# UCSC-nanopore-cgl/margin

Measured on AMD Instinct MI355X. Metric: het-sites x reads phased/sec (30x ONT synthetic chunks, end to end: every merge level + final sweep), higher is better.
Workload: dtype int32

## Files before the change

### include/margin_rphmm.h

```cpp
#ifndef MARGIN_RPHMM_H_
#define MARGIN_RPHMM_H_

#include <stddef.h>
#include <stdint.h>

#ifdef __cplusplus
extern "C" {
#endif

#define MRP_OK 0
#define MRP_ERR_ARG 1
#define MRP_ERR_NO_DEVICE 2
#define MRP_ERR_HIP 3
#define MRP_ERR_NOMEM 4
#define MRP_ERR_UNSUPPORTED 5
#define MRP_ERR_LOOKUP 6

#define MRP_ALLELE_LOG_PROB_BITS 8
#define MRP_MAX_READ_PARTITIONING_DEPTH 64
#define MRP_MAX_ALLELES 16

#define MRP_FLAG_MAX_NOT_SUM 1u
#define MRP_FLAG_INCLUDE_ANCESTOR_SUB_PROB 2u

// ... 1 lines not shown
typedef struct mrp_chunk mrp_chunk;
typedef struct mrp_batch mrp_batch;

const char *mrp_last_error(void);
const char *mrp_version(void);
#define MRP_ABI_VERSION 6
int mrp_abi_version(void);
int mrp_device_count(void);

int mrp_context_create(int device, mrp_context **out);
void mrp_context_destroy(mrp_context *ctx);
int mrp_context_synchronize(mrp_context *ctx);
int mrp_context_trim(mrp_context *ctx);
int mrp_runtime_init(void);
int mrp_context_set_phase_groups(mrp_context *ctx, int groups);
int mrp_context_set_test_hooks(mrp_context *ctx, int hooks);
int mrp_set_host_threads(int n);

int mrp_chunk_create(mrp_context *ctx, int64_t n_sites, const uint32_t *allele_number,
                     const uint16_t *substitution_log_probs, const uint16_t *allele_prior_log_probs,
                     const uint8_t *profile_pool, int64_t pool_bytes, mrp_chunk **out);
void mrp_chunk_destroy(mrp_chunk *chunk);

typedef struct mrp_hmm_job {
    const mrp_chunk *chunk;
    int32_t n_columns;
    uint32_t flags;
    const int32_t *col_ref_start;
    const int32_t *col_length;
    const int32_t *col_depth;
// ... 552 lines not shown
```

### margin_amd/capi.py

```python
from __future__ import annotations

import ctypes as C
import os
import time
from typing import Dict, List, Optional, Sequence

import numpy as np

_HERE = os.path.dirname(os.path.abspath(__file__))
LIB_PATH = os.environ.get("MRP_LIB_OVERRIDE") or os.path.join(_HERE, "lib", "libmargin_rphmm.so")

MRP_OK = 0
MRP_ERR_ARG, MRP_ERR_NO_DEVICE, MRP_ERR_HIP, MRP_ERR_NOMEM, MRP_ERR_UNSUPPORTED, MRP_ERR_LOOKUP = 1, 2, 3, 4, 5, 6
WIDE_MAX_WIDTH, WIDE_MAX_CELLS = 32768, 1 << 31
FLAG_MAX_NOT_SUM = 1
FLAG_INCLUDE_ANCESTOR_SUB_PROB = 2

ABI_VERSION = 6

EXPORTED_SYMBOLS = [
    "mrp_last_error", "mrp_version", "mrp_abi_version", "mrp_runtime_init", "mrp_device_count", "mrp_context_create", "mrp_context_destroy",
    "mrp_context_synchronize", "mrp_context_trim", "mrp_hmm_split", "mrp_hmm_split_where_phasing_is_uncertain", "mrp_context_set_phase_groups", "mrp_context_set_test_hooks", "mrp_set_host_threads", "mrp_chunk_create", "mrp_chunk_destroy", "mrp_fb_run", "mrp_batch_create",
    "mrp_batch_add", "mrp_batch_upload", "mrp_batch_launch", "mrp_batch_download", "mrp_batch_destroy",
    "mrp_batch_stats", "mrp_count_bit_vectors", "mrp_emissions", "mrp_get_rp_hmms", "mrp_hmm_destroy", "mrp_free",
    "mrp_hmm_view", "mrp_hmm_forward_backward", "mrp_hmm_prune", "mrp_hmm_forward_trace_back", "mrp_phase_reads",
    "mrp_phase_result_destroy", "mrp_get_rp_hmms_resident", "mrp_phase_reads_many", "mrp_reference_from_bubbles",
    "mrp_profile_seqs_from_bubbles", "mrp_assign_reads_to_haplotypes", "mrp_stitch_create", "mrp_stitch_destroy",
    "mrp_stitch_chunk", "mrp_stitch_size", "mrp_stitch_lookup", "mrp_phase_sets", "mrp_binomial_p_value", "mrp_binomial_coefficient",
    "mrp_symbols_from_chars", "mrp_pair_hmm_reverse_complement", "mrp_band_diagonals", "mrp_forward_probabilities",
    "mrp_allele_read_supports", "mrp_kmer_alignment_anchors", "mrp_phase_chunks_on_devices", "mrp_queue_plan", "mrp_queue_dry_run", "mrp_queue_create", "mrp_queue_destroy",
    "mrp_queue_phase_chunks", "mrp_partition_reads_by_haplotype", "mrp_phase_variants_from_tagged_reads", "mrp_phase_string_chunks",
    "mrp_extract_read_substrings", "mrp_string_chunk_from_extracted", "mrp_string_chunk_units", "mrp_queue_phase_string_chunks",
    "mrp_phase_string_chunks_on_devices", "mrp_phase_string_chunks_with_filtered", "mrp_queue_phase_string_chunks_with_filtered",
    "mrp_phase_string_chunks_with_filtered_on_devices", "mrp_haptag_sites_from_extracted", "mrp_haplotag_aligned_chunks",
    "mrp_kmer_alignment_anchors_many", "mrp_phase_aligned_chunks", "mrp_string_chunk_rest_from_extracted", "mrp_equal_substring_classes",
    "mrp_phase_aligned_chunks_with_filtered", "mrp_aligned_chunk_units", "mrp_queue_phase_aligned_chunks",
    "mrp_queue_phase_aligned_chunks_with_filtered", "mrp_phase_aligned_chunks_on_devices", "mrp_phase_aligned_chunks_with_filtered_on_devices",
# ... 269 lines not shown
    vp, i64, i32, u32 = C.c_void_p, C.c_int64, C.c_int32, C.c_uint32
    P = C.POINTER
    L.mrp_last_error.restype = C.c_char_p
    L.mrp_version.restype = C.c_char_p
    L.mrp_abi_version.restype = C.c_int
    if L.mrp_abi_version() != ABI_VERSION:
        raise MrpError(f"libmargin_rphmm.so speaks ABI {L.mrp_abi_version()}, this binding was transcribed from ABI {ABI_VERSION} of include/margin_rphmm.h")
    L.mrp_device_count.restype = C.c_int
    L.mrp_context_create.argtypes = [C.c_int, P(vp)]
    L.mrp_context_destroy.argtypes = [vp]
    L.mrp_context_destroy.restype = None
    L.mrp_context_synchronize.argtypes = [vp]
    L.mrp_context_trim.argtypes = [vp]
    L.mrp_context_set_phase_groups.argtypes = [vp, C.c_int]
    L.mrp_context_set_test_hooks.argtypes = [vp, C.c_int]
    L.mrp_set_host_threads.argtypes = [C.c_int]
    L.mrp_chunk_create.argtypes = [vp, i64, vp, vp, vp, vp, i64, P(vp)]
    L.mrp_chunk_destroy.argtypes = [vp]
    L.mrp_chunk_destroy.restype = None
    L.mrp_fb_run.argtypes = [vp, i64, P(HmmJob)]
    L.mrp_batch_create.argtypes = [vp, P(vp)]
    L.mrp_batch_add.argtypes = [vp, P(HmmJob)]
    L.mrp_batch_upload.argtypes = [vp]
    L.mrp_batch_launch.argtypes = [vp]
    L.mrp_batch_download.argtypes = [vp]
    L.mrp_batch_destroy.argtypes = [vp]
    L.mrp_batch_destroy.restype = None
    L.mrp_batch_stats.argtypes = [vp, P(LaunchStats)]
    L.mrp_count_bit_vectors.argtypes = [vp, vp, i32, i32, i32, vp, vp]
    L.mrp_emissions.argtypes = [vp, vp, i32, i32, i32, vp, u32, i64, vp, vp]
# ... 99 lines not shown
    def __init__(self, device: int = 0):
        L = load()
        h = C.c_void_p()
        _check(L.mrp_context_create(device, C.byref(h)))
        self.h = h

    def synchronize(self):
        _check(load().mrp_context_synchronize(self.h))

    def trim(self):
        _check(load().mrp_context_trim(self.h))

    def set_phase_groups(self, groups: int):
        _check(load().mrp_context_set_phase_groups(self.h, groups))

    def set_test_hooks(self, hooks: int):
        _check(load().mrp_context_set_test_hooks(self.h, hooks))

    def set_wide_pairs(self, on):
        _check(load().mrp_context_set_wide_pairs(self.h, int(bool(on))))

    def wide_pair_count(self):
        pairs, cells = C.c_int64(), C.c_int64()
        _check(load().mrp_context_wide_pair_count(self.h, C.byref(pairs), C.byref(cells)))
        return pairs.value, cells.value

    def close(self):
        if self.h:
            load().mrp_context_destroy(self.h)
            self.h = None
# ... 1400 lines not shown
```

### margin_amd/csrc/mrp_batch.cpp

```cpp
#include <hip/hip_runtime.h>

#include <algorithm>
#include <array>
#include <cstdio>
#include <cstdlib>
#include <cstring>
#include <ctime>
#include <mutex>
#include <new>
#include <vector>

#include "mrp_internal.h"
#include "mrp_level_order.h"

extern "C" {

int mrp_batch_create(mrp_context *ctx, mrp_batch **out) {
    if (!ctx || !out) return mrp_set_error(MRP_ERR_ARG, "mrp_batch_create: bad arguments");
    mrp_batch *b = new (std::nothrow) mrp_batch();
    if (!b) return mrp_set_error(MRP_ERR_NOMEM, "out of host memory");
    b->ctx = ctx;
    b->bind_pool(&ctx->pool);
    *out = b;
    return MRP_OK;
// ... 361 lines not shown
    HostVec<uint32_t>().swap(b->cell_next);
    HostVec<uint32_t>().swap(b->cell_prev);
    HostVec<uint32_t>().swap(b->cell_np);
    b->uploaded = true;
    return MRP_OK;
}

int mrp_batch_launch(mrp_batch *b) {
    if (!b) return mrp_set_error(MRP_ERR_ARG, "batch is NULL");
    if (!b->uploaded) {
        int rc = mrp_batch_upload(b);
        if (rc != MRP_OK) return rc;
    }
    mrp_context *ctx = b->ctx;
    HIP_TRY(hipSetDevice(ctx->device));
    hipStream_t s = ctx->stream;
    const MrpBatchDev &d = b->dev;
    hipStream_t ps = s;
    const size_t slot = (size_t) (b->n_launches % mrp_batch::EV_RING);
    if (slot >= b->ev_ring.size()) {
        std::array<hipEvent_t, 5> fresh{};
        for (auto &ev : fresh) HIP_TRY(hipEventCreate(&ev));
        b->ev_ring.push_back(fresh);
    }
    const std::array<hipEvent_t, 5> &ev = b->ev_ring[slot];
    if (b->n_launches >= mrp_batch::EV_RING) HIP_TRY(hipEventSynchronize(ev[2]));
    if (ps != s && ctx->last_emission) HIP_TRY(hipStreamWaitEvent(ps, ctx->last_emission, 0));
    HIP_TRY(hipEventRecord(ev[0], ps));
    HIP_TRY(mrp_launch_planes(d, ps));
    if (b->resident && mrp_dup('p')) HIP_TRY(mrp_launch_planes(d, ps));
    HIP_TRY(hipEventRecord(ev[1], ps));
// ... 266 lines not shown
```

### margin_amd/csrc/mrp_context.cpp

```cpp
#include <hip/hip_runtime.h>

#include <atomic>
#include <cstdarg>
#include <cstdio>
#include <cstdlib>
#include <mutex>
#include <new>

#include "mrp_internal.h"

static thread_local char g_err[512] = "";

extern "C" {

int mrp_set_error(int code, const char *fmt, ...) {
    va_list ap;
    va_start(ap, fmt);
    vsnprintf(g_err, sizeof(g_err), fmt, ap);
    va_end(ap);
    return code;
}

const char *mrp_last_error(void) { return g_err; }
const char *mrp_version(void) { return "margin_rphmm 0.5.0 gfx950"; }
int mrp_abi_version(void) { return MRP_ABI_VERSION; }

int mrp_runtime_init(void) {
    return MRP_OK;
}

int mrp_device_count(void) {
    int n = 0;
    if (hipGetDeviceCount(&n) != hipSuccess) return 0;
    return n;
}

int mrp_context_device(const mrp_context *ctx) { return ctx->device; }
void mrp_warn_hw_queues_once(int concurrent_batches) {
    static std::atomic<int> said{0};
    if (concurrent_batches <= 2 || getenv("MRP_QUIET")) return;
    const char *q = getenv("GPU_MAX_HW_QUEUES");
    const int have = q ? atoi(q) : 4;
    if (have >= 2 * concurrent_batches || have >= 16) return;
    if (said.exchange(1)) return;
    fprintf(stderr, "margin_rphmm: %d concurrent batches (two streams each) on %d hardware queues (GPU_MAX_HW_QUEUES%s): their kernels share "
                    "queues and serialize (MRP_QUIET silences this line)\n",
            concurrent_batches, have, q ? "" : " unset, the runtime's default");
}

int mrp_context_set_grouped(mrp_context *ctx, int grouped) { const int was = ctx->grouped ? 1 : 0; ctx->grouped = grouped != 0; return was; }
void mrp_context_set_concurrent_batches(mrp_context *ctx, int n) { ctx->concurrent_batches = n < 1 ? 1 : n; }
int mrp_context_calls_sharing_device(const mrp_context *ctx) { return ctx->calls_sharing_device; }
int64_t mrp_context_device_budget(mrp_context *ctx) {
    if (ctx->pool.device < 0 || hipSetDevice(ctx->device) != hipSuccess) return 0;
    const size_t b = DevPoolRegistry::get().budget_of(ctx->pool.device);
    return b > (size_t) 1 << 62 ? 0 : (int64_t) b;
}
// ... 3 lines not shown
    for (mrp_context *s_ : ctx->siblings) n += s_->pool.oom_local.load();
    return n;
}
void mrp_context_pool_bytes(mrp_context *ctx, int64_t *cached, int64_t *device_held) {
    { std::lock_guard<std::mutex> lock(ctx->pool.mu); *cached = (int64_t) ctx->pool.cached_bytes; }
    *device_held = ctx->pool.device >= 0 ? (int64_t) DevPoolRegistry::get().held[ctx->pool.device].load() : 0;
}
mrp_context *mrp_context_sibling(mrp_context *ctx, int i) {
    std::lock_guard<std::mutex> lock(ctx->sibling_mu);
    while ((int) ctx->siblings.size() <= i) {
        mrp_context *s = nullptr;
        if (mrp_context_create(ctx->device, &s) != MRP_OK) return nullptr;
        s->phase_groups = 1;
        s->grouped = true;
        s->test_hooks = ctx->test_hooks;
        ctx->siblings.push_back(s);
    }
    return ctx->siblings[(size_t) i];
}
int mrp_context_create(int device, mrp_context **out) {
    if (!out) return mrp_set_error(MRP_ERR_ARG, "mrp_context_create: out is NULL");
    *out = nullptr;
    int n = mrp_device_count();
    if (n <= 0) return mrp_set_error(MRP_ERR_NO_DEVICE, "no HIP device visible: the stRPHmm sweep has no CPU fallback");
    if (device < 0 || device >= n) return mrp_set_error(MRP_ERR_ARG, "device %d out of range (0..%d)", device, n - 1);
    HIP_TRY(hipSetDevice(device));
    mrp_context *ctx = new (std::nothrow) mrp_context();
    if (!ctx) return mrp_set_error(MRP_ERR_NOMEM, "out of host memory");
    ctx->device = device;
    ctx->pool.attach(device);
// ... 51 lines not shown
int mrp_context_set_phase_groups(mrp_context *ctx, int groups) {
    if (!ctx || groups < 0 || groups > 16) return mrp_set_error(MRP_ERR_ARG, "mrp_context_set_phase_groups: bad arguments");
    ctx->phase_groups = groups;
    return MRP_OK;
}
int mrp_context_phase_groups(const mrp_context *ctx) { return ctx->phase_groups; }
int mrp_context_set_test_hooks(mrp_context *ctx, int hooks) {
    if (!ctx || hooks < 0 || hooks > 127) return mrp_set_error(MRP_ERR_ARG, "mrp_context_set_test_hooks: bad arguments");
    if ((hooks & 4) && ctx->pool.device >= 0) DevPoolRegistry::get().inject_oom[ctx->pool.device].store(1);
    hooks &= ~4;
    ctx->test_hooks = hooks;
    for (mrp_context *s_ : ctx->siblings) s_->test_hooks = hooks;
    return MRP_OK;
}
int mrp_context_test_hooks(const mrp_context *ctx) { return ctx->test_hooks; }
int mrp_context_set_wide_pairs(mrp_context *ctx, int on) {
    if (!ctx) return mrp_set_error(MRP_ERR_ARG, "mrp_context_set_wide_pairs: context is NULL");
    ctx->wide_pairs = on != 0;
    return MRP_OK;
}
int mrp_context_wide_pair_count(mrp_context *ctx, int64_t *pairs_out, int64_t *cells_out) {
    if (!ctx) return mrp_set_error(MRP_ERR_ARG, "mrp_context_wide_pair_count: context is NULL");
    if (pairs_out) *pairs_out = ctx->wide_pair_count;
    if (cells_out) *cells_out = ctx->wide_cell_count;
    return MRP_OK;
}

}
```

### margin_amd/csrc/mrp_engine.cpp

```cpp
#include <hip/hip_runtime.h>

#include <cmath>
#include <cstdio>
#include <cstdlib>
#include <cstring>
#include <ctime>
#include <memory>
#include <new>
#include <vector>

#include "mrp_engine.h"
extern "C" void mrp_pool_set_tag(int t);
extern "C" void mrp_pool_set_weight(int ns_per_index);
#include "mrp_internal.h"
#include "mrp_level_order.h"

#define ENG_TRY(expr)                                                                                          \
    do {                                                                                                       \
        hipError_t e_ = (expr);                                                                                \
        if (e_ != hipSuccess) return mrp_set_error(MRP_ERR_HIP, "%s failed: %s", #expr, hipGetErrorString(e_)); \
    } while (0)

namespace {
struct Segment {
// ... 68 lines not shown
    void reset() { arrays.release(); on = false; }
};
}

struct mrp_engine_level_state {
    mrp_batch *b = nullptr;
    std::unique_ptr<Segment> seg;
    int seg_id = -1;
    mrp_xhmm *x = nullptr;
    int64_t n = 0;
    bool final_level = false;
    bool fused = false;
    bool units = false;
    bool any_pack = true, any_planes = true;
    bool deferred = false;
    HmmIndex ix;
    LevelOrder order;
    PruneParams pp{};
    DevBufGroup arrays;
    DevBuf<PlanCol> d_plan{arrays};
    DevBuf<XDesc> d_xd{arrays};
    DevBuf<mrp_xpar> d_par{arrays};
    DevBuf<int32_t> d_cstart{arrays}, d_croff{arrays};
    DevBuf<PlanHmm> d_phmm{arrays};
    DevBuf<uint16_t> d_dims{arrays};
    DevBuf<LayoutTot> d_tot{arrays};
    DevBuf<LayoutBase> d_base{arrays};
    DevBuf<int64_t> d_totals{arrays}, d_tile_sums{arrays};
    DevBuf<CrossCol> d_cc{arrays};
    DevBuf<PruneHmm> d_ph{arrays};
// ... 13 lines not shown
    hipError_t create_events() {
        hipError_t he = hipEventCreateWithFlags(&done, hipEventDisableTiming);
        if (he == hipSuccess) he = hipEventCreate(&lay0);
        if (he == hipSuccess) he = hipEventCreateWithFlags(&uploaded, hipEventDisableTiming);
        for (auto &e_ : ev)
            if (he == hipSuccess) he = hipEventCreate(&e_);
        return he;
    }
    void reset() {
        seg.reset();
        arrays.release();
        frag.reset();
        order.perm.clear();
        x = nullptr; n = 0;
        deferred = false;
        t = Timing{};
    }
    ~mrp_engine_level_state() {
        for (hipEvent_t e_ : {uploaded, done, lay0, ev[0], ev[1], ev[2], ev[3], ev[4]})
            if (e_) (void) hipEventDestroy(e_);
        if (b) mrp_batch_destroy(b);
    }
};

struct mrp_engine {
    mrp_context *ctx = nullptr;
    mrp_params params{};
    PruneParams pp{};
    DevBufGroup arrays;
    DevBuf<uint64_t> leaf_part{arrays};
// ... 17 lines not shown
};

static double eng_now() {
    timespec ts;
    clock_gettime(CLOCK_MONOTONIC, &ts);
    return 1e3 * ts.tv_sec + 1e-6 * ts.tv_nsec;
}

static int64_t level_bound_bytes(const mrp_engine_level_state *L) { return 16 * L->order.bound_cells + 8 * L->order.bound_merge; }

static void level_retire(mrp_engine *e, mrp_engine_level_state *L, bool complete = false) {
    if (!L) return;
    mrp_context *ctx = e->ctx;
    (void) hipSetDevice(ctx->device);
    if (!complete) {
        (void) ctx->wait_stream(ctx->stream);
        if (ctx->pre) (void) ctx->wait_stream(ctx->pre);
    }
    if (L->b) {
        L->b->recycle();
        e->spare.push_back(L->b);
        L->b = nullptr;
    }
    if (L->deferred) e->inflight_bytes -= level_bound_bytes(L);
    L->reset();
    e->spare_levels.push_back(L);
    ctx->pool.reclaim();
}

extern "C" {

int mrp_engine_create(mrp_context *ctx, const mrp_params *params, mrp_engine **out) {
    if (!ctx || !params || !out) return mrp_set_error(MRP_ERR_ARG, "mrp_engine_create: NULL argument");
    *out = nullptr;
    if (params->reserved != 0) return mrp_set_error(MRP_ERR_ARG, "mrp_params.reserved must be 0");
    if (!params->max_not_sum_transitions)
        return mrp_set_error(MRP_ERR_UNSUPPORTED, "the device-resident merge needs maxNotSumTransitions (integer posteriors)");
    const int64_t lim = std::max<int64_t>(params->min_partitions_in_a_column, params->max_partitions_in_a_column);
    if (lim < 1 || lim > MRP_PRUNE_MAX_S || params->min_partitions_in_a_column < 0)
        return mrp_set_error(MRP_ERR_UNSUPPORTED, "the device-resident merge keeps at most %d partitions per column", MRP_PRUNE_MAX_S);
    ENG_TRY(hipSetDevice(ctx->device));
    mrp_engine *e = new (std::nothrow) mrp_engine();
// ... 403 lines not shown
        if (n1 < 0 || n2 < 0 || n1 > cap || n2 > cap) return;
        memcpy(h.frag_sites, h_sites + f.site0, sizeof(FragSite) * (size_t) f.length);
        memcpy(h.frag_reads1, h_lists + 2 * f.list0, 4 * (size_t) n1);
        memcpy(h.frag_reads2, h_lists + 2 * f.list0 + cap, 4 * (size_t) n2);
        h.frag_n1 = n1; h.frag_n2 = n2; h.frag_done = 1;
    });
}

static int level_stage(mrp_engine *e, int64_t n, mrp_xhmm *x, bool final_level) {
    if (!e || n < 0 || (n > 0 && !x)) return mrp_set_error(MRP_ERR_ARG, "mrp_engine_level: bad arguments");
    if (e->staged) return mrp_set_error(MRP_ERR_ARG, "mrp_engine_level_stage: a staged level was not launched");
    if (n == 0) return MRP_OK;
    mrp_context *ctx = e->ctx;
    ENG_TRY(hipSetDevice(ctx->device));
    hipStream_t cs = nullptr;
    ENG_TRY(ctx->copy_stream(&cs));
    if (e->n_segs >= mrp_engine::MAX_SEGS) return mrp_set_error(MRP_ERR_UNSUPPORTED, "more than %d levels", mrp_engine::MAX_SEGS);
    std::unique_ptr<mrp_engine_level_state> L;
    int rc = level_take(e, n, x, final_level, L);
    if (rc != MRP_OK) return rc;
    L->t.begin = eng_now();
    L->x = x;
    L->n = n;
    L->final_level = final_level;
    L->fused = !final_level && !(ctx->test_hooks & 2);
    for (int64_t i = 0; i < n && L->fused; i++)
        if (x[i].flags & MRP_FLAG_INCLUDE_ANCESTOR_SUB_PROB) L->fused = false;
    L->units = L->fused && e->pp.pairs != 0 && !(ctx->test_hooks & (8 | 16));

    double tm[5];
    bool all_planes = true;
    tm[0] = eng_now();
    if ((rc = level_index(e, L.get(), cs, &all_planes)) != MRP_OK) return rc;
    tm[1] = eng_now();
    if ((rc = level_segment(e, L.get())) != MRP_OK) return rc;
    tm[2] = eng_now();
// ... 98 lines not shown
    if (rc == MRP_OK) {
        if (Lp->final_level) level_scatter_final(Lp);
        level_book_stats(e, Lp);
        e->segments.push_back(std::move(Lp->seg));
    }
    e->n_ended++;
    level_retire(e, Lp, complete);
    return rc;
}

static int level_finish(mrp_engine *e) {
    if (e->inflight.empty()) return MRP_OK;
    mrp_context *ctx = e->ctx;
    int rc = MRP_OK;
    hipError_t se = hipSetDevice(ctx->device);
    if (se == hipSuccess) se = ctx->wait_stream(ctx->stream);
    if (se != hipSuccess) rc = mrp_set_error(MRP_ERR_HIP, "hipStreamSynchronize failed: %s", hipGetErrorString(se));
    std::vector<mrp_engine_level_state *> all;
    all.swap(e->inflight);
    for (auto *Lp : all) {
        if (rc == MRP_OK) rc = level_finish_one(e, Lp, false);
        else { e->n_ended++; level_retire(e, Lp); }
    }
    return rc;
}

static int level_finish_ready(mrp_engine *e) {
    int rc = MRP_OK;
    while (rc == MRP_OK && !e->inflight.empty()) {
        mrp_engine_level_state *Lp = e->inflight.front();
        if (!Lp->done || hipEventQuery(Lp->done) != hipSuccess) { (void) hipGetLastError(); break; }
        e->inflight.erase(e->inflight.begin());
        rc = level_finish_one(e, Lp, true);
    }
    return rc;
}

static int launch_layout(mrp_engine *e, mrp_engine_level_state *L, hipStream_t s) {
    mrp_batch *b = L->b;
    LayoutOut lo{};
    lo.dims = L->d_dims.p; lo.tot = L->d_tot.p; lo.base = L->d_base.p; lo.totals = L->d_totals.p; lo.tile_sums = L->d_tile_sums.p;
    lo.hmms = b->d_hmms.p; lo.cols = b->d_cols.p; lo.scols = b->d_scols.p; lo.pcols = b->d_pcols.p; lo.tilecols = b->d_tilecols.p;
    lo.ccols = L->d_cc.p;
    ENG_TRY(hipStreamWaitEvent(s, L->uploaded, 0));
    ENG_TRY(hipEventRecord(L->lay0, s));
    ENG_TRY_DUP('l', mrp_launch_layout(L->d_plan.p, L->d_phmm.p, L->n, L->ix.total_cols, b->d_chunks.p, e->pp.S,
                                       (e->params.include_inverted_partitions ? MRP_XF_INVERTED : 0u) | (L->units ? MRP_XF_UNITS : 0u), lo, s));
    ENG_TRY(hipMemcpyAsync(L->res.totals, L->d_totals.p, 48, hipMemcpyDeviceToHost, s));
    return MRP_OK;
}

static constexpr int64_t DEFER_BYTES = (int64_t) 1024 << 20;
static constexpr size_t DEFER_LEVELS = 12;
static bool level_defers(const mrp_engine *e, const mrp_engine_level_state *L) {
    const int64_t bound_bytes = level_bound_bytes(L);
    return !(e->ctx->test_hooks & 32) && L->fused && !L->final_level && bound_bytes <= DEFER_BYTES &&
           e->inflight_bytes + bound_bytes <= 4 * DEFER_BYTES && e->inflight.size() < DEFER_LEVELS;
}

static int launch_size_batch(mrp_engine_level_state *L, int64_t cells, int64_t merge, int64_t tiles_fast, int64_t tiles) {
    mrp_batch *b = L->b;
    const int64_t n = L->n, total_cols = L->ix.total_cols, n_slots = L->ix.total_slots;
    b->n_cells_total = cells; b->n_merge = merge; b->n_slots = n_slots; b->n_tiles_dev = tiles; b->n_fast_tiles = tiles_fast;
    b->stats.n_cells = cells; b->stats.n_merge_cells = merge;
    b->stats.algorithmic_bytes = 24 * cells + 32 * merge + 8 * total_cols;
    const size_t nC = (size_t) cells;
    if (L->fused) { b->d_partition.release(); b->n_tiles_dev = 0; b->n_fast_tiles = 0; }
    else ENG_TRY(b->d_partition.alloc(nC));
    ENG_TRY(b->d_np.alloc(nC)); ENG_TRY(b->d_cost.alloc(nC));
    ENG_TRY(b->d_f32.alloc(nC)); ENG_TRY(b->d_b32.alloc(nC));
    ENG_TRY(b->d_mf32.alloc((size_t) merge)); ENG_TRY(b->d_mb32.alloc((size_t) merge));
    if (!L->fused) ENG_TRY(b->d_tiles.alloc((size_t) tiles));
// ... 63 lines not shown
        if (L->frag.on) { const int rc = L->frag.fetch(n, s); if (rc != MRP_OK) return rc; }
    }
    ENG_TRY(hipMemcpyAsync(L->res.err, L->d_err.p, 16, hipMemcpyDeviceToHost, s));
    ENG_TRY(hipMemcpyAsync(L->res.err_hmm, L->d_err_hmm.p, sizeof(int32_t) * (size_t) n, hipMemcpyDeviceToHost, s));
#if defined(PRUNE_EXP_CLOCK) || defined(PRUNE_EXP_CLOCK2) || defined(XE_CLOCK)
    ENG_TRY(hipMemcpyAsync(L->clk, L->d_err.p + 4, 96, hipMemcpyDeviceToHost, s));
#endif
    ENG_TRY(hipEventRecord(L->done, s));
    return MRP_OK;
}

static int level_launch_impl(mrp_engine *e, mrp_engine_level_state *L) {
    mrp_context *ctx = e->ctx;
    ENG_TRY(hipSetDevice(ctx->device));
    hipStream_t s = ctx->stream;
    const double t0 = eng_now();
    int rc = launch_layout(e, L, s);
    if (rc != MRP_OK) return rc;
    int64_t cells, merge, tiles_fast = 0, tiles = 0;
    if (level_defers(e, L)) {
        if ((rc = level_finish_ready(e)) != MRP_OK) return rc;
        cells = L->order.bound_cells; merge = L->order.bound_merge;
        L->deferred = true;
        e->inflight_bytes += level_bound_bytes(L);
    } else {
        if ((rc = level_finish(e)) != MRP_OK) return rc;
        ENG_TRY(ctx->wait_stream(s));
        L->t.react_ms = -eng_now();
        ctx->pool.reclaim();
        const int64_t *tot = L->res.totals;
// ... 35 lines not shown
```

### margin_amd/csrc/mrp_internal.h

```cpp
#ifndef MRP_INTERNAL_H_
#define MRP_INTERNAL_H_

#include <hip/hip_runtime.h>
#include <cstring>
#include <cstdlib>

#include <time.h>

#include <algorithm>
#include <array>
#include <atomic>
#include <functional>
#include <iterator>
#include <map>
#include <memory>
#include <new>
#include <type_traits>
#include <mutex>
#include <thread>
#include <utility>
#include <vector>

#include "../../include/margin_rphmm.h"
#include "mrp_device.h"
// ... 64 lines not shown
        }
        return b;
    }
    void forget_budget(int device) { if (device >= 0 && device < MAX_DEVICES) budget[device].store(0, std::memory_order_relaxed); }
    void shrink_budget(int device) {
        const size_t ours = held[device].load(std::memory_order_relaxed);
        size_t b = budget[device].load(std::memory_order_relaxed);
        if (ours > ((size_t) 1 << 30) && (b == 0 || ours < b)) budget[device].store(ours, std::memory_order_relaxed);
    }
    inline void trim_device(int device, DevPool *but);
};

struct DevPool {
    std::mutex mu;
    std::multimap<size_t, void *> free_blocks;
    std::vector<std::pair<size_t, void *>> pending;
    size_t cached_bytes = 0;
    size_t cache_limit = (size_t) 64 << 30;
    int device = -1;
    std::atomic<uint64_t> oom_local{0};
    void attach(int dev) {
        device = dev >= 0 && dev < DevPoolRegistry::MAX_DEVICES ? dev : -1;
        if (device < 0) return;
        DevPoolRegistry &r = DevPoolRegistry::get();
        std::lock_guard<std::mutex> lock(r.mu);
        r.pools.push_back(this);
    }
    void detach() {
        if (device < 0) return;
        DevPoolRegistry &r = DevPoolRegistry::get();
        std::lock_guard<std::mutex> lock(r.mu);
// ... 48 lines not shown
        if (e != hipSuccess && device >= 0) {
            (void) hipGetLastError();
            DevPoolRegistry::get().trim_device(device, this);
            e = hipMalloc(p, cls);
        }
        if (e == hipSuccess) held_add(cls);
        else if (e == hipErrorOutOfMemory && device >= 0) {
            DevPoolRegistry::get().oom_events[device].fetch_add(1, std::memory_order_relaxed);
            oom_local.fetch_add(1, std::memory_order_relaxed);
            DevPoolRegistry::get().shrink_budget(device);
        }
        return e;
    }
    void release(void *p, size_t cls) {
        std::lock_guard<std::mutex> lock(mu);
        pending.emplace_back(cls, p);
    }
    void reclaim() {
        std::lock_guard<std::mutex> lock(mu);
        for (auto &b : pending) {
            free_blocks.emplace(b.first, b.second);
            cached_bytes += b.first;
        }
        pending.clear();
        while ((cached_bytes > cache_limit || over_budget()) && !free_blocks.empty()) {
            auto it = std::prev(free_blocks.end());
            (void) hipFree(it->second);
            held_sub(it->first);
            cached_bytes -= it->first;
            free_blocks.erase(it);
        }
    }
    void trim() {
        std::lock_guard<std::mutex> lock(mu);
        for (auto &b : free_blocks) { (void) hipFree(b.second); held_sub(b.first); }
        free_blocks.clear();
        cached_bytes = 0;
    }
    void destroy() {
// ... 48 lines not shown
            (void) hipDeviceSynchronize();
            e = hipMemset(p, 0xA5, bytes);
            (void) hipDeviceSynchronize();
        }
#endif
        return e;
    }
    template <class A>
    hipError_t upload(const std::vector<T, A> &h, hipStream_t s) {
        hipError_t e = alloc(h.size());
        if (e != hipSuccess || h.empty()) return e;
        return hipMemcpyAsync(p, h.data(), h.size() * sizeof(T), hipMemcpyHostToDevice, s);
    }
};

struct mrp_context {
    int device = 0;
    hipStream_t stream = nullptr;
    hipStream_t aux[2] = {nullptr, nullptr};
    bool grouped = false;
    int concurrent_batches = 1;
    int calls_sharing_device = 1;
    hipError_t side_streams(hipStream_t *a0, hipStream_t *a1) {
        if (grouped) { *a0 = *a1 = stream; return hipSuccess; }
        for (int i = 0; i < 2; i++)
            if (!aux[i]) { const hipError_t e = hipStreamCreateWithFlags(&aux[i], hipStreamNonBlocking); if (e != hipSuccess) return e; }
        *a0 = aux[0]; *a1 = aux[1];
        return hipSuccess;
    }
    hipError_t copy_stream(hipStream_t *cs) {
        if (!pre) { const hipError_t e = hipStreamCreateWithFlags(&pre, hipStreamNonBlocking); if (e != hipSuccess) return e; }
        *cs = pre;
        return hipSuccess;
// ... 8 lines not shown
        timespec c0, c1, w0, w1;
        clock_gettime(CLOCK_THREAD_CPUTIME_ID, &c0); clock_gettime(CLOCK_MONOTONIC, &w0);
        const hipError_t e = wait_stream_impl(s);
        clock_gettime(CLOCK_THREAD_CPUTIME_ID, &c1); clock_gettime(CLOCK_MONOTONIC, &w1);
        wait_cpu_ms += 1e3 * (c1.tv_sec - c0.tv_sec) + 1e-6 * (c1.tv_nsec - c0.tv_nsec);
        wait_wall_ms += 1e3 * (w1.tv_sec - w0.tv_sec) + 1e-6 * (w1.tv_nsec - w0.tv_nsec);
        return e;
    }
    hipError_t wait_stream_impl(hipStream_t s) {
        if (!block_ev) {
            hipError_t e = hipEventCreateWithFlags(&block_ev, hipEventDisableTiming);
            if (e != hipSuccess) { block_ev = nullptr; return hipStreamSynchronize(s); }
        }
        hipError_t e = hipEventRecord(block_ev, s);
        if (e != hipSuccess) return e;
        for (;;) {
            e = hipEventQuery(block_ev);
            if (e != hipErrorNotReady) return e;
            timespec ts{0, 30000};
            nanosleep(&ts, nullptr);
        }
    }
    DevPool pool;
    int test_hooks = 0;
    int wide_pairs = 0;
    int64_t wide_pair_count = 0, wide_cell_count = 0;
    int phase_groups = 0;
    std::vector<mrp_context *> siblings;
    std::mutex sibling_mu;
    std::vector<struct mrp_engine_level_state *> spare_levels;
    std::vector<struct mrp_batch *> spare_batches;
};

struct mrp_chunk {
    mrp_context *ctx = nullptr;
    int64_t n_sites = 0, pool_bytes = 0;
// ... 60 lines not shown
struct mrp_batch {
    mrp_context *ctx = nullptr;
    std::mutex mu;
    std::vector<const mrp_chunk *> chunks;
    HostVec<DevHmm> hmms;
    HostVec<DevCol> cols;
    HostVec<int64_t> read_byte_off;
    HostVec<uint64_t> partition;
    HostVec<SweepCol> scols;
    HostVec<PlaneCol> pcols;
    HostVec<uint32_t> cell_next, cell_prev, cell_np;
    HostVec<EmitTile> tiles;
    int64_t n_fast_tiles = 0;
    int64_t n_tiles_dev = 0;
    std::function<hipError_t(hipStream_t)> pre_sweep;
    DevBufGroup arrays;
    DevBuf<TileCol> d_tilecols{arrays};
    bool need_wide = false;
    std::vector<JobOut> outs;
    int64_t n_merge = 0, n_slots = 0;
    int64_t n_cells_total = 0;
    bool resident = false;
    mrp_launch_stats stats{};
    std::vector<int32_t> order_wide, order_mid, order_narrow, order_f64, order_lse, order_lse_big, order_gen;
    int max_merge_wide = 1, max_merge_mid = 1, max_merge_narrow = 1, max_merge_lse = 1, max_merge_lse_big = 1;
    bool uploaded = false, launched = false;
    static constexpr int EV_RING = 32;
    std::vector<std::array<hipEvent_t, 5>> ev_ring;
    int64_t n_launches = 0, stats_mark = 0;
    DevBuf<DevHmm> d_hmms{arrays};
// ... 7 lines not shown
    DevBuf<double> d_f{arrays}, d_b{arrays}, d_mf{arrays}, d_mb{arrays}, d_total{arrays}, d_hmm_fb{arrays};
    DevBuf<int32_t> d_f32{arrays}, d_b32{arrays}, d_mf32{arrays}, d_mb32{arrays};
    DevBuf<int32_t> d_order_wide{arrays}, d_order_mid{arrays}, d_order_narrow{arrays}, d_order_f64{arrays}, d_order_lse{arrays}, d_order_lse_big{arrays},
        d_pack_list{arrays}, d_plane_list{arrays};
    DevBuf<EmitTile> d_tiles{arrays};
    MrpBatchDev dev{};
    void recycle() {
        arrays.release();
        chunks.clear(); hmms.clear(); cols.clear(); read_byte_off.clear(); partition.clear(); scols.clear(); pcols.clear();
        cell_next.clear(); cell_prev.clear(); cell_np.clear(); tiles.clear(); outs.clear();
        order_wide.clear(); order_mid.clear(); order_narrow.clear(); order_f64.clear(); order_lse.clear(); order_lse_big.clear(); order_gen.clear();
        n_fast_tiles = 0; n_tiles_dev = 0; need_wide = false; n_merge = 0; n_slots = 0; n_cells_total = 0; resident = false;
        stats = mrp_launch_stats{};
        max_merge_wide = max_merge_mid = max_merge_narrow = max_merge_lse = max_merge_lse_big = 1;
        uploaded = launched = false;
        n_launches = 0; stats_mark = 0;
        dev = MrpBatchDev{};
    }
    void bind_pool(DevPool *pl) { arrays.bind(pl); }
    MrpBatchDev view() const {
        MrpBatchDev d{};
        d.hmms = d_hmms.p; d.cols = d_cols.p; d.scols = d_scols.p; d.pcols = d_pcols.p; d.chunks = d_chunks.p; d.read_byte_off = d_read_byte_off.p;
        d.pack_list = d_pack_list.p; d.plane_list = d_plane_list.p; d.n_pack_list = (int64_t) d_pack_list.n; d.n_plane_list = (int64_t) d_plane_list.n;
        d.partition = d_partition.p; d.cell_np = d_np.p; d.cell_next = d_next.p; d.cell_prev = d_prev.p;
        d.planes = d_planes.p; d.slot_total = d_slot_total.p; d.slot_bytes = d_slot_bytes.p; d.cell_cost = d_cost.p;
        d.cell_f32 = d_f32.p; d.cell_b32 = d_b32.p; d.merge_f32 = d_mf32.p; d.merge_b32 = d_mb32.p;
        d.cell_f = d_f.p; d.cell_b = d_b.p; d.merge_f = d_mf.p; d.merge_b = d_mb.p; d.col_total = d_total.p; d.hmm_fb = d_hmm_fb.p;
        d.n_hmms = (int64_t) hmms.size(); d.n_cols = (int64_t) cols.size(); d.n_cells = n_cells_total; d.n_merge = n_merge; d.n_slots = n_slots;
        return d;
    }
// ... 105 lines not shown
```

### margin_amd/csrc/rphmm_host.h

```cpp
#ifndef RPHMM_HOST_H_
#define RPHMM_HOST_H_

#include <stdint.h>

#include "../../include/margin_rphmm.h"

#ifdef __cplusplus
extern "C" {
#endif

typedef struct mrp_chunk_host {
    int64_t n_sites;
    const uint32_t *allele_number;
    const uint32_t *allele_offset;
    const uint32_t *sub_offset;
    const uint16_t *sub;
    const uint16_t *prior;
    const uint8_t *pool;
    int64_t pool_bytes;
} mrp_chunk_host;

void mrp_chunk_host_view(const mrp_chunk *chunk, mrp_chunk_host *out);
mrp_context *mrp_chunk_context(const mrp_chunk *chunk);
void mrp_phase_group_assign(int64_t n_chunks, int G, int64_t total_sites, uint8_t *group_of);
int mrp_context_device(const mrp_context *ctx);
int mrp_context_set_grouped(mrp_context *ctx, int grouped);
void mrp_context_set_concurrent_batches(mrp_context *ctx, int n);
int mrp_context_calls_sharing_device(const mrp_context *ctx);
void mrp_context_pool_bytes(mrp_context *ctx, int64_t *cached, int64_t *device_held);
void mrp_warn_hw_queues_once(int concurrent_batches);
uint64_t mrp_context_oom_events(mrp_context *ctx);
int64_t mrp_context_device_budget(mrp_context *ctx);
mrp_context *mrp_context_sibling(mrp_context *ctx, int i);
int mrp_set_error(int code, const char *fmt, ...);
int mrp_host_threads(void);
int mrp_context_phase_groups(const mrp_context *ctx);
int mrp_phase_groups_for(const mrp_context *ctx, int64_t n_chunks);
int mrp_context_test_hooks(const mrp_context *ctx);
void mrp_pool_set_priority(int p);
void mrp_pool_set_tag(int t);
void *mrp_pool_current(void);
void mrp_pool_adopt(void *pool);
long long mrp_pool_tag_cpu_ns(int tag);
void mrp_pool_run(int64_t n, int64_t grain, void (*fn)(int64_t, void *), void *arg);
void mrp_pool_set_weight(int ns_per_index);
// ... 73 lines not shown
```

### margin_amd/csrc/rphmm_many.c

```c
#define _GNU_SOURCE
#include "rphmm_common.h"

typedef struct {
    mrp_context *ctx;
    int64_t n;
    const mrp_chunk **chunks;
    const mrp_read **reads;
    int64_t *n_reads;
    const mrp_params *params;
    mrp_phase_result **out;
    mrp_phase_many_stats stats;
    int rc, index;
    void *pool;
    char err[256];
} phase_group;
long long mrp_pool_task_cpu_ns(void);
long long mrp_pool_task_cpu_ns_this_thread(void);
static double thread_cpu_ms(void) { struct timespec t; clock_gettime(CLOCK_THREAD_CPUTIME_ID, &t); return 1e3 * t.tv_sec + 1e-6 * t.tv_nsec; }
void mrp_phase_group_assign(int64_t n_chunks, int G, int64_t total_sites, uint8_t *group_of) {
    int w[16], W = 0, pat[256], np = 0;
    if (G < 1) G = 1;
    if (G > 16) G = 16;
    const int graded = G >= 4 && n_chunks >= 16 * (int64_t) G && total_sites >= 500 * n_chunks;
    for (int g = 0; g < G; g++) w[g] = graded ? (g + 2 < 5 ? g + 2 : 5) : 1;
// ... 96 lines not shown
            q->ctx = g == 0 ? ctx : mrp_context_sibling(ctx, g - 1);
            q->params = params;
            q->n = 0;
            for (int64_t i = 0; i < n_chunks; i++) if (group_of[i] == g) q->n++;
            q->chunks = xmalloc(sizeof(*q->chunks) * (size_t) (q->n + 1));
            q->reads = xmalloc(sizeof(*q->reads) * (size_t) (q->n + 1));
            q->n_reads = xmalloc(sizeof(*q->n_reads) * (size_t) (q->n + 1));
            q->out = xcalloc((size_t) q->n + 1, sizeof(*q->out));
            q->n = 0;
            for (int64_t i = 0; i < n_chunks; i++)
                if (group_of[i] == g) { q->chunks[q->n] = chunks[i]; q->reads[q->n] = reads[i]; q->n_reads[q->n] = n_reads[i]; q->n++; }
            if (!q->ctx) { q->rc = MRP_ERR_HIP; snprintf(q->err, sizeof(q->err), "%s", mrp_last_error()); }
        }
        const int was_grouped = mrp_context_set_grouped(ctx, 1);
        for (int g = 0; g < G; g++) if (grp[g].ctx) mrp_context_set_concurrent_batches(grp[g].ctx, G * mrp_context_calls_sharing_device(ctx));
        mrp_warn_hw_queues_once(G);
        for (int g = 1; g < G; g++)
            if (grp[g].ctx && pthread_create(&th[g], NULL, phase_group_main, &grp[g]) == 0) started[g] = 1;
        if (grp[0].ctx) phase_group_main(&grp[0]);
        for (int g = 1; g < G; g++) {
            if (started[g]) pthread_join(th[g], NULL);
            else if (grp[g].ctx) phase_group_main(&grp[g]);
        }
        mrp_context_set_grouped(ctx, was_grouped);
        for (int g = 0; g < G; g++) if (grp[g].ctx) mrp_context_set_concurrent_batches(grp[g].ctx, 1);
        for (int g = 0; g < G; g++) {
            phase_group *q = &grp[g];
            if (q->rc != MRP_OK && (rc == MRP_OK || rc == MRP_ERR_UNSUPPORTED)) rc = mrp_set_error(q->rc, "%s", q->err);
            { int64_t k = 0; for (int64_t i = 0; i < n_chunks; i++) if (group_of[i] == g) out[i] = q->out[k++]; }
            if (stats && q->rc == MRP_OK) { stats_add(stats, &q->stats, first); first = 0; }
            free(q->chunks); free(q->reads); free(q->n_reads); free(q->out);
        }
        free(grp);
        free(group_of);
    }
    if (rc == MRP_ERR_UNSUPPORTED) {
        char why[160];
        snprintf(why, sizeof(why), "%s", mrp_last_error());
// ... 88 lines not shown
```

Measured before the change: 425.0 million.

## Add shared device lanes that schedule phase-group levels across streams by load

Adds an opt-in 'device lanes' mode. The streams of all phase-group sibling contexts become a shared pool, and each fused level launch goes to the least-loaded stream, with event waits keeping levels in order. The aim is to avoid oversubscribing the hardware queues when many groups each own two streams. Device-pool reclamation is now tagged per level, so retiring one level frees only its own blocks instead of every pending block. Defer limits become runtime-settable. Lanes stay off unless enabled, so the default path mostly changes only pool reclamation and the source of the defer constants.

```diff
diff --git a/include/margin_rphmm.h b/include/margin_rphmm.h
--- a/include/margin_rphmm.h
+++ b/include/margin_rphmm.h
@@ -39,6 +39,8 @@
 int mrp_context_trim(mrp_context *ctx);
 int mrp_runtime_init(void);
 int mrp_context_set_phase_groups(mrp_context *ctx, int groups);
+int mrp_context_set_device_lanes(mrp_context *ctx, int n);
+int mrp_context_set_defer_limits(mrp_context *ctx, int64_t bytes, int levels);
 int mrp_context_set_test_hooks(mrp_context *ctx, int hooks);
 int mrp_set_host_threads(int n);
 
diff --git a/margin_amd/capi.py b/margin_amd/capi.py
--- a/margin_amd/capi.py
+++ b/margin_amd/capi.py
@@ -20,7 +20,7 @@
 
 EXPORTED_SYMBOLS = [
     "mrp_last_error", "mrp_version", "mrp_abi_version", "mrp_runtime_init", "mrp_device_count", "mrp_context_create", "mrp_context_destroy",
-    "mrp_context_synchronize", "mrp_context_trim", "mrp_hmm_split", "mrp_hmm_split_where_phasing_is_uncertain", "mrp_context_set_phase_groups", "mrp_context_set_test_hooks", "mrp_set_host_threads", "mrp_chunk_create", "mrp_chunk_destroy", "mrp_fb_run", "mrp_batch_create",
+    "mrp_context_synchronize", "mrp_context_trim", "mrp_hmm_split", "mrp_hmm_split_where_phasing_is_uncertain", "mrp_context_set_phase_groups", "mrp_context_set_device_lanes", "mrp_context_set_defer_limits", "mrp_context_set_test_hooks", "mrp_set_host_threads", "mrp_chunk_create", "mrp_chunk_destroy", "mrp_fb_run", "mrp_batch_create",
     "mrp_batch_add", "mrp_batch_upload", "mrp_batch_launch", "mrp_batch_download", "mrp_batch_destroy",
     "mrp_batch_stats", "mrp_count_bit_vectors", "mrp_emissions", "mrp_get_rp_hmms", "mrp_hmm_destroy", "mrp_free",
     "mrp_hmm_view", "mrp_hmm_forward_backward", "mrp_hmm_prune", "mrp_hmm_forward_trace_back", "mrp_phase_reads",
@@ -320,6 +320,9 @@
     L.mrp_context_trim.argtypes = [vp]
     L.mrp_context_set_phase_groups.argtypes = [vp, C.c_int]
     L.mrp_context_set_test_hooks.argtypes = [vp, C.c_int]
+    if hasattr(L, "mrp_context_set_device_lanes"):
+        L.mrp_context_set_device_lanes.argtypes = [vp, C.c_int]
+        L.mrp_context_set_defer_limits.argtypes = [vp, i64, C.c_int]
     L.mrp_set_host_threads.argtypes = [C.c_int]
     L.mrp_chunk_create.argtypes = [vp, i64, vp, vp, vp, vp, i64, P(vp)]
     L.mrp_chunk_destroy.argtypes = [vp]
@@ -449,6 +452,12 @@
     def set_phase_groups(self, groups: int):
         _check(load().mrp_context_set_phase_groups(self.h, groups))
 
+    def set_device_lanes(self, n: int):
+        _check(load().mrp_context_set_device_lanes(self.h, n))
+
+    def set_defer_limits(self, nbytes: int, levels: int):
+        _check(load().mrp_context_set_defer_limits(self.h, nbytes, levels))
+
     def set_test_hooks(self, hooks: int):
         _check(load().mrp_context_set_test_hooks(self.h, hooks))
 
diff --git a/margin_amd/csrc/mrp_batch.cpp b/margin_amd/csrc/mrp_batch.cpp
--- a/margin_amd/csrc/mrp_batch.cpp
+++ b/margin_amd/csrc/mrp_batch.cpp
@@ -399,7 +399,7 @@
     }
     mrp_context *ctx = b->ctx;
     HIP_TRY(hipSetDevice(ctx->device));
-    hipStream_t s = ctx->stream;
+    hipStream_t s = b->lane ? b->lane : ctx->stream;
     const MrpBatchDev &d = b->dev;
     hipStream_t ps = s;
     const size_t slot = (size_t) (b->n_launches % mrp_batch::EV_RING);
diff --git a/margin_amd/csrc/mrp_context.cpp b/margin_amd/csrc/mrp_context.cpp
--- a/margin_amd/csrc/mrp_context.cpp
+++ b/margin_amd/csrc/mrp_context.cpp
@@ -36,11 +36,46 @@
 }
 
 int mrp_context_device(const mrp_context *ctx) { return ctx->device; }
+int mrp_hw_queues_granted(void) {
+    const char *q = getenv("GPU_MAX_HW_QUEUES");
+    const int have = q ? atoi(q) : 4;
+    return have < 1 ? 1 : have > 32 ? 32 : have;
+}
+int mrp_lane_pick(const int64_t *load, int n_lanes) {
+    int best = 0;
+    for (int i = 1; i < n_lanes; i++)
+        if (load[i] < load[best]) best = i;
+    return best;
+}
+int mrp_context_lanes_begin(mrp_context *root, int G) {
+    if (!root) return 0;
+    root->last_lanes = 0;
+    if (G < 2 || root->device_lanes == 0) return 0;
+    const int Q = root->device_lanes > 0 ? root->device_lanes : mrp_hw_queues_granted();
+    if (2 * G <= Q) return 0;
+    std::lock_guard<std::mutex> lock(root->sibling_mu);
+    if ((int) root->siblings.size() < G - 1) return 0;
+    mrp_lanes &ln = root->lanes_store;
+    ln.n = std::min(std::min(Q, G), (int) mrp_lanes::MAX);
+    for (int i = 0; i < ln.n; i++) { ln.stream[i] = i == 0 ? root->stream : root->siblings[(size_t) i - 1]->stream; ln.load[i] = 0; }
+    if (hipSetDevice(root->device) != hipSuccess || root->copy_stream(&ln.copy) != hipSuccess) { (void) hipGetLastError(); return 0; }
+    root->lanes = &ln;
+    for (int g = 1; g < G; g++) root->siblings[(size_t) g - 1]->lanes = &ln;
+    root->last_lanes = ln.n;
+    return ln.n;
+}
+int mrp_context_last_lanes(const mrp_context *ctx) { return ctx ? ctx->last_lanes : 0; }
+void mrp_context_lanes_end(mrp_context *root, int G) {
+    if (!root) return;
+    std::lock_guard<std::mutex> lock(root->sibling_mu);
+    root->lanes = nullptr;
+    for (int g = 1; g < G && g - 1 < (int) root->siblings.size(); g++) root->siblings[(size_t) g - 1]->lanes = nullptr;
+}
 void mrp_warn_hw_queues_once(int concurrent_batches) {
     static std::atomic<int> said{0};
     if (concurrent_batches <= 2 || getenv("MRP_QUIET")) return;
     const char *q = getenv("GPU_MAX_HW_QUEUES");
-    const int have = q ? atoi(q) : 4;
+    const int have = mrp_hw_queues_granted();
     if (have >= 2 * concurrent_batches || have >= 16) return;
     if (said.exchange(1)) return;
     fprintf(stderr, "margin_rphmm: %d concurrent batches (two streams each) on %d hardware queues (GPU_MAX_HW_QUEUES%s): their kernels share "
@@ -74,6 +109,7 @@
         s->phase_groups = 1;
         s->grouped = true;
         s->test_hooks = ctx->test_hooks;
+        s->defer_bytes = ctx->defer_bytes; s->defer_levels = ctx->defer_levels;
         ctx->siblings.push_back(s);
     }
     return ctx->siblings[(size_t) i];
@@ -155,6 +191,18 @@
     return MRP_OK;
 }
 int mrp_context_test_hooks(const mrp_context *ctx) { return ctx->test_hooks; }
+int mrp_context_set_device_lanes(mrp_context *ctx, int n) {
+    if (!ctx || n < -1 || n > mrp_lanes::MAX) return mrp_set_error(MRP_ERR_ARG, "mrp_context_set_device_lanes: bad arguments");
+    ctx->device_lanes = n;
+    return MRP_OK;
+}
+int mrp_context_set_defer_limits(mrp_context *ctx, int64_t bytes, int levels) {
+    if (!ctx || bytes < 0 || levels < 0 || levels > 32) return mrp_set_error(MRP_ERR_ARG, "mrp_context_set_defer_limits: bad arguments");
+    std::lock_guard<std::mutex> lock(ctx->sibling_mu);
+    ctx->defer_bytes = bytes; ctx->defer_levels = levels;
+    for (mrp_context *s_ : ctx->siblings) { s_->defer_bytes = bytes; s_->defer_levels = levels; }
+    return MRP_OK;
+}
 int mrp_context_set_wide_pairs(mrp_context *ctx, int on) {
     if (!ctx) return mrp_set_error(MRP_ERR_ARG, "mrp_context_set_wide_pairs: context is NULL");
     ctx->wide_pairs = on != 0;
diff --git a/margin_amd/csrc/mrp_engine.cpp b/margin_amd/csrc/mrp_engine.cpp
--- a/margin_amd/csrc/mrp_engine.cpp
+++ b/margin_amd/csrc/mrp_engine.cpp
@@ -106,6 +106,11 @@
     bool units = false;
     bool any_pack = true, any_planes = true;
     bool deferred = false;
+    uint64_t seq = 0;
+    hipStream_t cs = nullptr, s = nullptr;
+    mrp_lanes *lanes = nullptr;
+    int lane = -1;
+    int64_t lane_load = 0;
     HmmIndex ix;
     LevelOrder order;
     PruneParams pp{};
@@ -149,6 +154,7 @@
         order.perm.clear();
         x = nullptr; n = 0;
         deferred = false;
+        cs = s = nullptr; lanes = nullptr; lane = -1; lane_load = 0;
         t = Timing{};
     }
     ~mrp_engine_level_state() {
@@ -196,9 +202,16 @@
     mrp_context *ctx = e->ctx;
     (void) hipSetDevice(ctx->device);
     if (!complete) {
-        (void) ctx->wait_stream(ctx->stream);
-        if (ctx->pre) (void) ctx->wait_stream(ctx->pre);
-    }
+        (void) ctx->wait_stream(L->s ? L->s : ctx->stream);
+        if (L->cs) (void) ctx->wait_stream(L->cs);
+        else if (ctx->pre) (void) ctx->wait_stream(ctx->pre);
+    }
+    if (L->lanes && L->lane >= 0) {
+        std::lock_guard<std::mutex> lock(L->lanes->mu);
+        L->lanes->load[L->lane] -= L->lane_load;
+    }
+    const uint64_t seq = L->seq;
+    ctx->pool.release_tag = seq;
     if (L->b) {
         L->b->recycle();
         e->spare.push_back(L->b);
@@ -206,8 +219,9 @@
     }
     if (L->deferred) e->inflight_bytes -= level_bound_bytes(L);
     L->reset();
+    ctx->pool.release_tag = 0;
     e->spare_levels.push_back(L);
-    ctx->pool.reclaim();
+    ctx->pool.reclaim_level(seq);
 }
 
 extern "C" {
@@ -641,12 +655,16 @@
     mrp_context *ctx = e->ctx;
     ENG_TRY(hipSetDevice(ctx->device));
     hipStream_t cs = nullptr;
-    ENG_TRY(ctx->copy_stream(&cs));
+    mrp_lanes *lanes = ctx->lanes;
+    if (lanes) cs = lanes->copy;
+    else ENG_TRY(ctx->copy_stream(&cs));
     if (e->n_segs >= mrp_engine::MAX_SEGS) return mrp_set_error(MRP_ERR_UNSUPPORTED, "more than %d levels", mrp_engine::MAX_SEGS);
     std::unique_ptr<mrp_engine_level_state> L;
     int rc = level_take(e, n, x, final_level, L);
     if (rc != MRP_OK) return rc;
     L->t.begin = eng_now();
+    L->seq = ++ctx->level_seq;
+    L->cs = cs; L->s = nullptr; L->lanes = lanes; L->lane = -1; L->lane_load = 0;
     L->x = x;
     L->n = n;
     L->final_level = final_level;
@@ -775,12 +793,13 @@
     mrp_context *ctx = e->ctx;
     int rc = MRP_OK;
     hipError_t se = hipSetDevice(ctx->device);
-    if (se == hipSuccess) se = ctx->wait_stream(ctx->stream);
+    const bool by_event = e->inflight.back()->lanes != nullptr;
+    if (se == hipSuccess) se = by_event ? ctx->wait_event(e->inflight.back()->done) : ctx->wait_stream(ctx->stream);
     if (se != hipSuccess) rc = mrp_set_error(MRP_ERR_HIP, "hipStreamSynchronize failed: %s", hipGetErrorString(se));
     std::vector<mrp_engine_level_state *> all;
     all.swap(e->inflight);
     for (auto *Lp : all) {
-        if (rc == MRP_OK) rc = level_finish_one(e, Lp, false);
+        if (rc == MRP_OK) rc = level_finish_one(e, Lp, by_event);
         else { e->n_ended++; level_retire(e, Lp); }
     }
     return rc;
@@ -811,12 +830,10 @@
     return MRP_OK;
 }
 
-static constexpr int64_t DEFER_BYTES = (int64_t) 1024 << 20;
-static constexpr size_t DEFER_LEVELS = 12;
 static bool level_defers(const mrp_engine *e, const mrp_engine_level_state *L) {
-    const int64_t bound_bytes = level_bound_bytes(L);
-    return !(e->ctx->test_hooks & 32) && L->fused && !L->final_level && bound_bytes <= DEFER_BYTES &&
-           e->inflight_bytes + bound_bytes <= 4 * DEFER_BYTES && e->inflight.size() < DEFER_LEVELS;
+    const int64_t bound_bytes = level_bound_bytes(L), defer_bytes = e->ctx->defer_bytes;
+    return !(e->ctx->test_hooks & 32) && L->fused && !L->final_level && bound_bytes <= defer_bytes &&
+           e->inflight_bytes + bound_bytes <= 4 * defer_bytes && e->inflight.size() < (size_t) e->ctx->defer_levels;
 }
 
 static int launch_size_batch(mrp_engine_level_state *L, int64_t cells, int64_t merge, int64_t tiles_fast, int64_t tiles) {
@@ -910,6 +927,18 @@
     mrp_context *ctx = e->ctx;
     ENG_TRY(hipSetDevice(ctx->device));
     hipStream_t s = ctx->stream;
+    if (mrp_lanes *ln = L->lanes) {
+        {
+            std::lock_guard<std::mutex> lock(ln->mu);
+            L->lane = mrp_lane_pick(ln->load, ln->n);
+            L->lane_load = std::max<int64_t>(1, L->order.bound_cells);
+            ln->load[L->lane] += L->lane_load;
+        }
+        s = ln->stream[L->lane];
+        L->b->lane = s;
+        if (!e->inflight.empty() && e->inflight.back()->s != s) ENG_TRY(hipStreamWaitEvent(s, e->inflight.back()->done, 0));
+    }
+    L->s = s;
     const double t0 = eng_now();
     int rc = launch_layout(e, L, s);
     if (rc != MRP_OK) return rc;
diff --git a/margin_amd/csrc/mrp_internal.h b/margin_amd/csrc/mrp_internal.h
--- a/margin_amd/csrc/mrp_internal.h
+++ b/margin_amd/csrc/mrp_internal.h
@@ -102,7 +102,9 @@
 struct DevPool {
     std::mutex mu;
     std::multimap<size_t, void *> free_blocks;
-    std::vector<std::pair<size_t, void *>> pending;
+    struct Pending { size_t cls; void *p; uint64_t tag; };
+    std::vector<Pending> pending;
+    uint64_t release_tag = 0;
     size_t cached_bytes = 0;
     size_t cache_limit = (size_t) 64 << 30;
     int device = -1;
@@ -181,15 +183,19 @@
     }
     void release(void *p, size_t cls) {
         std::lock_guard<std::mutex> lock(mu);
-        pending.emplace_back(cls, p);
-    }
-    void reclaim() {
+        pending.push_back({cls, p, release_tag});
+    }
+    void reclaim() { reclaim_tagged(0, true); }
+    void reclaim_level(uint64_t tag) { reclaim_tagged(tag, false); }
+    void reclaim_tagged(uint64_t tag, bool all) {
         std::lock_guard<std::mutex> lock(mu);
+        size_t kept = 0;
         for (auto &b : pending) {
-            free_blocks.emplace(b.first, b.second);
-            cached_bytes += b.first;
-        }
-        pending.clear();
+            if (!all && b.tag != tag) { pending[kept++] = b; continue; }
+            free_blocks.emplace(b.cls, b.p);
+            cached_bytes += b.cls;
+        }
+        pending.resize(kept);
         while ((cached_bytes > cache_limit || over_budget()) && !free_blocks.empty()) {
             auto it = std::prev(free_blocks.end());
             (void) hipFree(it->second);
@@ -268,9 +274,25 @@
     }
 };
 
+struct mrp_lanes {
+    static constexpr int MAX = 32;
+    int n = 0;
+    hipStream_t stream[MAX] = {nullptr};
+    hipStream_t copy = nullptr;
+    std::mutex mu;
+    int64_t load[MAX] = {0};
+};
+
 struct mrp_context {
     int device = 0;
     hipStream_t stream = nullptr;
+    mrp_lanes *lanes = nullptr;
+    mrp_lanes lanes_store;
+    int device_lanes = 0;
+    int last_lanes = 0;
+    int64_t defer_bytes = (int64_t) 1024 << 20;
+    int defer_levels = 12;
+    uint64_t level_seq = 0;
     hipStream_t aux[2] = {nullptr, nullptr};
     bool grouped = false;
     int concurrent_batches = 1;
@@ -309,12 +331,24 @@
         }
         hipError_t e = hipEventRecord(block_ev, s);
         if (e != hipSuccess) return e;
+        return poll_event(block_ev);
+    }
+    static hipError_t poll_event(hipEvent_t ev) {
         for (;;) {
-            e = hipEventQuery(block_ev);
+            const hipError_t e = hipEventQuery(ev);
             if (e != hipErrorNotReady) return e;
             timespec ts{0, 30000};
             nanosleep(&ts, nullptr);
         }
+    }
+    hipError_t wait_event(hipEvent_t ev) {
+        timespec c0, c1, w0, w1;
+        clock_gettime(CLOCK_THREAD_CPUTIME_ID, &c0); clock_gettime(CLOCK_MONOTONIC, &w0);
+        const hipError_t e = poll_event(ev);
+        clock_gettime(CLOCK_THREAD_CPUTIME_ID, &c1); clock_gettime(CLOCK_MONOTONIC, &w1);
+        wait_cpu_ms += 1e3 * (c1.tv_sec - c0.tv_sec) + 1e-6 * (c1.tv_nsec - c0.tv_nsec);
+        wait_wall_ms += 1e3 * (w1.tv_sec - w0.tv_sec) + 1e-6 * (w1.tv_nsec - w0.tv_nsec);
+        return e;
     }
     DevPool pool;
     int test_hooks = 0;
@@ -405,6 +439,7 @@
     int64_t n_fast_tiles = 0;
     int64_t n_tiles_dev = 0;
     std::function<hipError_t(hipStream_t)> pre_sweep;
+    hipStream_t lane = nullptr;
     DevBufGroup arrays;
     DevBuf<TileCol> d_tilecols{arrays};
     bool need_wide = false;
@@ -442,6 +477,7 @@
         stats = mrp_launch_stats{};
         max_merge_wide = max_merge_mid = max_merge_narrow = max_merge_lse = max_merge_lse_big = 1;
         uploaded = launched = false;
+        lane = nullptr;
         n_launches = 0; stats_mark = 0;
         dev = MrpBatchDev{};
     }
diff --git a/margin_amd/csrc/rphmm_host.h b/margin_amd/csrc/rphmm_host.h
--- a/margin_amd/csrc/rphmm_host.h
+++ b/margin_amd/csrc/rphmm_host.h
@@ -29,6 +29,11 @@
 int mrp_context_calls_sharing_device(const mrp_context *ctx);
 void mrp_context_pool_bytes(mrp_context *ctx, int64_t *cached, int64_t *device_held);
 void mrp_warn_hw_queues_once(int concurrent_batches);
+int mrp_hw_queues_granted(void);
+int mrp_context_lanes_begin(mrp_context *root, int G);
+void mrp_context_lanes_end(mrp_context *root, int G);
+int mrp_context_last_lanes(const mrp_context *ctx);
+int mrp_lane_pick(const int64_t *load, int n_lanes);
 uint64_t mrp_context_oom_events(mrp_context *ctx);
 int64_t mrp_context_device_budget(mrp_context *ctx);
 mrp_context *mrp_context_sibling(mrp_context *ctx, int i);
diff --git a/margin_amd/csrc/rphmm_many.c b/margin_amd/csrc/rphmm_many.c
--- a/margin_amd/csrc/rphmm_many.c
+++ b/margin_amd/csrc/rphmm_many.c
@@ -134,7 +134,10 @@
         }
         const int was_grouped = mrp_context_set_grouped(ctx, 1);
         for (int g = 0; g < G; g++) if (grp[g].ctx) mrp_context_set_concurrent_batches(grp[g].ctx, G * mrp_context_calls_sharing_device(ctx));
-        mrp_warn_hw_queues_once(G);
+        int all_ctx = 1;
+        for (int g = 0; g < G; g++) if (!grp[g].ctx) all_ctx = 0;
+        const int lanes = all_ctx ? mrp_context_lanes_begin(ctx, G) : 0;
+        if (!lanes) mrp_warn_hw_queues_once(G);
         for (int g = 1; g < G; g++)
             if (grp[g].ctx && pthread_create(&th[g], NULL, phase_group_main, &grp[g]) == 0) started[g] = 1;
         if (grp[0].ctx) phase_group_main(&grp[0]);
@@ -142,6 +145,7 @@
             if (started[g]) pthread_join(th[g], NULL);
             else if (grp[g].ctx) phase_group_main(&grp[g]);
         }
+        if (lanes) mrp_context_lanes_end(ctx, G);
         mrp_context_set_grouped(ctx, was_grouped);
         for (int g = 0; g < G; g++) if (grp[g].ctx) mrp_context_set_concurrent_batches(grp[g].ctx, 1);
         for (int g = 0; g < G; g++) {
```

After: 417.1 million. -1.9%, worse.
